# PaoPaoRobot/ygz-slam

Measured on AMD Instinct MI355X. Metric: frames/sec (extract+match+LK+local-BA), 640x480, 1000 ORB kpts; frames resident in HBM (PCIe-inclusive rate: value_with_transfers), higher is better.
Workload: dtype u8/f32/f64; 1 GPU; 2x640x480-pair pipeline: ORB extract + 256-bit Hamming BF cross-check + KLT 21x21x5 + FindDirectProjection + SparseImgAlign + local-BA 10x2000 linearise, per frame; resident_batches_per_gpu=1

## Files before the change

### ygz_slam_amd/csrc/image.hip

```cpp
#include "ygz_internal.h"
#include <limits.h>

__device__ __forceinline__ uint32_t gray1(uint32_t b, uint32_t g, uint32_t r)
{
    return (1868u * b + 9617u * g + 4899u * r + 8192u) >> 14;
}

typedef uint32_t img_u32x4 __attribute__((ext_vector_type(4)));
typedef img_u32x4 __attribute__((aligned(4))) img_u32x4u;
typedef img_u32x4 __attribute__((aligned(1))) img_u32x4b;
typedef uint32_t __attribute__((aligned(1))) img_u32b;
__global__ __launch_bounds__(256) void k_bgr2gray16(const uint8_t *__restrict__ bgr, uint8_t *__restrict__ gray,
                                                    unsigned npix, int slot_begin, uint8_t *__restrict__ pad, int width, int height)
{
    const unsigned i = blockIdx.x * 256u + threadIdx.x;
    if (i * 16u >= npix) return;
    const size_t slot = (size_t)(slot_begin + blockIdx.y);
    const uint4 *src = reinterpret_cast<const uint4 *>(bgr + slot * npix * 3u) + (size_t)i * 3u;
    const uint4 a = src[0], b = src[1], c = src[2];
    const uint32_t w[12] = { a.x, a.y, a.z, a.w, b.x, b.y, b.z, b.w, c.x, c.y, c.z, c.w };
    uint32_t out[4];
#pragma unroll
    for (int q = 0; q < 4; ++q) {
        const uint32_t w0 = w[3 * q], w1 = w[3 * q + 1], w2 = w[3 * q + 2];
        const uint32_t g0 = gray1(w0 & 255u, (w0 >> 8) & 255u, (w0 >> 16) & 255u);
        const uint32_t g1 = gray1(w0 >> 24, w1 & 255u, (w1 >> 8) & 255u);
        const uint32_t g2 = gray1((w1 >> 16) & 255u, w1 >> 24, w2 & 255u);
        const uint32_t g3 = gray1((w2 >> 8) & 255u, (w2 >> 16) & 255u, w2 >> 24);
        out[q] = g0 | (g1 << 8) | (g2 << 16) | (g3 << 24);
    }
    reinterpret_cast<uint4 *>(gray + slot * npix)[i] = make_uint4(out[0], out[1], out[2], out[3]);
    if (pad) {
        const unsigned p0 = i * 16u, y = p0 / (unsigned)width, x = p0 - y * (unsigned)width;
        const size_t pw = (size_t)KLT_PW(width), ph = (size_t)height + 2 * KLT_B;
        uint8_t *base = pad + slot * pw * ph;
        img_u32x4 v; v.x = out[0]; v.y = out[1]; v.z = out[2]; v.w = out[3];
        const uint32_t r0 = __builtin_amdgcn_perm(out[0], out[0], 0x00010203u), r1 = __builtin_amdgcn_perm(out[1], out[1], 0x00010203u),
                       r2 = __builtin_amdgcn_perm(out[2], out[2], 0x00010203u), r3 = __builtin_amdgcn_perm(out[3], out[3], 0x00010203u);
        img_u32x4 rv; rv.x = r3; rv.y = r2; rv.z = r1; rv.w = r0;
        auto store_row = [&](int r) {
            uint8_t *row = base + (size_t)r * pw;
            *reinterpret_cast<img_u32x4u *>(row + x + KLT_B) = v;
            if (x == 0u) *reinterpret_cast<img_u32x4b *>(row + KLT_B - 15) = rv;
            else if (x == 16u) {
                *reinterpret_cast<img_u32b *>(row + 5) = r0; *reinterpret_cast<img_u32b *>(row + 1) = r1; row[0] = (uint8_t)(out[2] & 255u);
            }
            if ((int)x == width - 16) *reinterpret_cast<img_u32x4b *>(row + KLT_B + width - 1) = rv;
            else if ((int)x == width - 32) {
                *reinterpret_cast<img_u32b *>(row + KLT_B + width + 15) = r3; *reinterpret_cast<img_u32b *>(row + KLT_B + width + 19) = r2;
                row[KLT_B + width + 23] = (uint8_t)(out[1] >> 24);
            }
        };
        store_row((int)y + KLT_B);
        if (y >= 1u && y <= (unsigned)KLT_B) store_row(KLT_B - (int)y);
        if ((int)y >= height - 1 - KLT_B && (int)y <= height - 2) store_row(KLT_B + 2 * (height - 1) - (int)y);
    }
}

__global__ __launch_bounds__(256) void k_bgr2gray1(const uint8_t *__restrict__ bgr, uint8_t *__restrict__ gray,
                                                   unsigned npix, int slot_begin)
{
    const unsigned i = blockIdx.x * 256u + threadIdx.x;
    if (i >= npix) return;
    const size_t slot = (size_t)(slot_begin + blockIdx.y);
    const uint8_t *s = bgr + (slot * npix + i) * 3u;
    gray[slot * npix + i] = (uint8_t)gray1(s[0], s[1], s[2]);
}

__device__ __forceinline__ int reflect101(int i, int n)
{
    if (n == 1) return 0;
    while (i < 0 || i >= n) i = (i < 0) ? -i : 2 * (n - 1) - i;
    return i;
}

#define PD_TW 64
#define PD_TH 32
#define PD_RPT (PD_TH / 4)
#define PD_SW 160
#define PD_SH (2 * PD_TH + 3)
#define PD_X0 16
__global__ __launch_bounds__(256) void k_pyr_down(const uint8_t *__restrict__ src, uint8_t *__restrict__ dst,
                                                  int sw, int sh, int dw, int dh, int slot_begin, uint8_t *__restrict__ pad, int frame_here)
{
    __shared__ __attribute__((aligned(16))) uint8_t tile[PD_SH][PD_SW];
    const size_t slot = (size_t)(slot_begin + blockIdx.z);
    const uint8_t *s = src + slot * (size_t)sw * sh;
    uint8_t *d = dst + slot * (size_t)dw * dh;
    const int dpw = KLT_PW(dw);
    uint8_t *pd = pad ? pad + slot * (size_t)dpw * (dh + 2 * KLT_B) + (size_t)KLT_B * dpw + KLT_B : nullptr;
    const int ox0 = blockIdx.x * PD_TW, oy0 = blockIdx.y * PD_TH;
    const int sx0 = 2 * ox0 - PD_X0, sy0 = 2 * oy0 - 2;
    const bool aligned = (sw & 15) == 0;
    constexpr int PD_RW = PD_SW / 16, PD_TOT = PD_SH * PD_RW, PD_N = (PD_TOT + 255) / 256;
    uint4 stage[PD_N];
#pragma unroll
    for (int k = 0; k < PD_N; ++k) {
        const int i = threadIdx.x + 256 * k;
        const int r = i / PD_RW, c16 = (i % PD_RW) * 16;
        uint4 v = make_uint4(0u, 0u, 0u, 0u);
        if (i < PD_TOT) {
            const int sy = reflect101(sy0 + r, sh), sx = sx0 + c16;
            const uint8_t *row = s + (size_t)sy * sw;
            if (aligned && sx >= 0 && sx + 15 < sw) v = *reinterpret_cast<const uint4 *>(row + sx);
            else {
                uint32_t w4[4];
#pragma unroll
                for (int q = 0; q < 4; ++q)
                    w4[q] = (uint32_t)row[reflect101(sx + 4 * q, sw)] | ((uint32_t)row[reflect101(sx + 4 * q + 1, sw)] << 8) |
                            ((uint32_t)row[reflect101(sx + 4 * q + 2, sw)] << 16) | ((uint32_t)row[reflect101(sx + 4 * q + 3, sw)] << 24);
                v = make_uint4(w4[0], w4[1], w4[2], w4[3]);
            }
        }
        stage[k] = v;
    }
#pragma unroll
    for (int k = 0; k < PD_N; ++k) {
        const int i = threadIdx.x + 256 * k;
        if (i < PD_TOT) *reinterpret_cast<uint4 *>(&tile[i / PD_RW][(i % PD_RW) * 16]) = stage[k];
    }
    __syncthreads();
    const int tx = threadIdx.x & 63, ty0 = (threadIdx.x >> 6) * PD_RPT;
    const int ox = ox0 + tx;
    int hrow[2 * PD_RPT + 3];
#pragma unroll
    for (int r = 0; r < 2 * PD_RPT + 3; ++r) {
        const uint32_t *tw = reinterpret_cast<const uint32_t *>(&tile[2 * ty0 + r][(2 * tx + PD_X0 - 2) & ~3]);
        const uint32_t d0 = tw[0], d1 = tw[1], sh = (uint32_t)((2 * tx + PD_X0 - 2) & 3);
        const uint32_t v4 = __builtin_amdgcn_alignbyte(d1, d0, sh);
        hrow[r] = (int)__builtin_amdgcn_udot4(v4, 0x04060401u, (d1 >> (8 * sh)) & 255u, false);
    }
    if (ox < dw) {
#pragma unroll
        for (int k = 0; k < PD_RPT; ++k) {
            const int oy = oy0 + ty0 + k;
            if (oy < dh) {
                const int v = hrow[2 * k] + 4 * hrow[2 * k + 1] + 6 * hrow[2 * k + 2] + 4 * hrow[2 * k + 3] + hrow[2 * k + 4];
                const uint8_t o8 = (uint8_t)((v + 128) >> 8);
                d[(size_t)oy * dw + ox] = o8;
                if (pd) {
                    pd[(size_t)oy * dpw + ox] = o8;
                    if (frame_here) {
                        const bool fl = ox >= 1 && ox <= KLT_B, fr = ox >= dw - 1 - KLT_B && ox <= dw - 2;
                        const bool ft = oy >= 1 && oy <= KLT_B, fb = oy >= dh - 1 - KLT_B && oy <= dh - 2;
                        if (fl | fr | ft | fb) {
                            const ptrdiff_t xl = -ox, xr = 2 * (dw - 1) - ox, yt = (ptrdiff_t)(-oy) * dpw, yb = (ptrdiff_t)(2 * (dh - 1) - oy) * dpw, y0 = (ptrdiff_t)oy * dpw;
                            if (fl) pd[y0 + xl] = o8;
                            if (fr) pd[y0 + xr] = o8;
                            if (ft) { pd[yt + ox] = o8; if (fl) pd[yt + xl] = o8; if (fr) pd[yt + xr] = o8; }
                            if (fb) { pd[yb + ox] = o8; if (fl) pd[yb + xl] = o8; if (fr) pd[yb + xr] = o8; }
                        }
                    }
                }
            }
        }
    }
}

struct FrameArgs {
    const uint8_t *img[YGZ_MAX_LEVELS]; uint8_t *pad[YGZ_MAX_LEVELS];
    int w[YGZ_MAX_LEVELS], h[YGZ_MAX_LEVELS];
    int first[YGZ_MAX_LEVELS], items[YGZ_MAX_LEVELS];
    int n_levels, slot_begin, full0;
};
typedef uint32_t __attribute__((aligned(1))) img_u32u;
__global__ __launch_bounds__(256) void k_klt_frame(FrameArgs A)
{
    int L = 0;
#pragma unroll
    for (int k = 1; k < YGZ_MAX_LEVELS; ++k) if (k < A.n_levels && (int)blockIdx.x >= A.first[k]) L = k;
    const int item = ((int)blockIdx.x - A.first[L]) * 256 + (int)threadIdx.x;
    if (item >= A.items[L]) return;
    const int w = A.w[L], h = A.h[L], pw = KLT_PW(w), ph = h + 2 * KLT_B, pw4 = pw >> 2;
    int y, dc;
    if (A.full0 && L == 0) { y = item / pw4; dc = item - y * pw4; }
    else {
        const int r0 = (KLT_B + w) >> 2, nr = pw4 - r0, band = KLT_B * pw4, mid = (KLT_B >> 2) + nr;
        if (item < band) { y = item / pw4; dc = item - y * pw4; }
        else if (item < 2 * band) { const int j = item - band; y = j / pw4; dc = j - y * pw4; y += KLT_B + h; }
        else {
            const int j = item - 2 * band;
            y = j / mid;
            const int c = j - y * mid;
            y += KLT_B;
            dc = c < (KLT_B >> 2) ? c : r0 + (c - (KLT_B >> 2));
        }
    }
    const size_t slot = (size_t)(A.slot_begin + (int)blockIdx.y);
    const uint8_t *row = A.img[L] + slot * (size_t)w * h + (size_t)reflect101(y - KLT_B, h) * w;
    const int x = 4 * dc - KLT_B;
    uint32_t v = 0;
    if (x >= 0 && x + 3 < w) v = *reinterpret_cast<const img_u32u *>(row + x);
    else {
#pragma unroll
        for (int k = 0; k < 4; ++k) v |= (uint32_t)row[reflect101(x + k, w)] << (8 * k);
    }
    *reinterpret_cast<uint32_t *>(A.pad[L] + slot * (size_t)pw * ph + (size_t)y * pw + 4 * dc) = v;
}

int ygz_launch_gray_pyramid(ygz_hip_ctx *ctx, int slot_begin, int n_slots, int from_bgr, int up_to_level)
{
    int rc = ygz_ensure_levels(ctx, up_to_level);
    if (rc != YGZ_OK) return rc;
    const unsigned npix = (unsigned)ctx->lw[0] * (unsigned)ctx->lh[0];
    int fuse_levels = 0;
    while (fuse_levels < up_to_level && ctx->klt_pad[fuse_levels]) ++fuse_levels;
    const bool fuse = fuse_levels > 0;
    const bool l0_framed = fuse && from_bgr && (npix & 15u) == 0 && (ctx->lw[0] & 15) == 0 && ctx->lw[0] >= 64 && ctx->lh[0] >= 2 * KLT_B + 2;
    bool framed[YGZ_MAX_LEVELS];
    for (int L = 0; L < YGZ_MAX_LEVELS; ++L) framed[L] = L == 0 ? l0_framed : (L < fuse_levels && ctx->lw[L] > KLT_B + 1 && ctx->lh[L] > KLT_B + 1);
    if (from_bgr) {
        if ((npix & 15u) == 0)
            YGZ_LAUNCH(ctx, KID_BGR2GRAY, k_bgr2gray16, dim3(ygz_div_up((int)(npix / 16), 256), n_slots), dim3(256),
                               ctx->bgr, ctx->lvl[0], npix, slot_begin, l0_framed ? ctx->klt_pad[0] : (uint8_t *)nullptr, ctx->lw[0], ctx->lh[0]);
        else
            YGZ_LAUNCH(ctx, KID_BGR2GRAY, k_bgr2gray1, dim3(ygz_div_up((int)npix, 256), n_slots), dim3(256),
                               ctx->bgr, ctx->lvl[0], npix, slot_begin);
    }
    for (int L = 1; L < up_to_level; ++L) {
        const int sw = ctx->lw[L - 1], sh = ctx->lh[L - 1], dw = ctx->lw[L], dh = ctx->lh[L];
        YGZ_LAUNCH(ctx, KID_PYR_DOWN, k_pyr_down, dim3(ygz_div_up(dw, PD_TW), ygz_div_up(dh, PD_TH), n_slots), dim3(256), ctx->lvl[L - 1], ctx->lvl[L], sw, sh, dw, dh, slot_begin,
                   L < fuse_levels ? ctx->klt_pad[L] : (uint8_t *)nullptr, framed[L] ? 1 : 0);
    }
    if (fuse) {
        FrameArgs F;
        for (int L = 0; L < YGZ_MAX_LEVELS; ++L) { F.img[L] = nullptr; F.pad[L] = nullptr; F.w[L] = F.h[L] = 0; F.first[L] = 0; F.items[L] = 0; }
        int total = 0;
        for (int L = 0; L < fuse_levels; ++L) {
            const int w = ctx->lw[L], h = ctx->lh[L], pw4 = KLT_PW(w) >> 2;
            F.img[L] = ctx->lvl[L]; F.pad[L] = ctx->klt_pad[L]; F.w[L] = w; F.h[L] = h;
            F.first[L] = total;
            F.items[L] = framed[L] ? 0 : (L == 0 ? pw4 * (h + 2 * KLT_B) : 2 * KLT_B * pw4 + h * ((KLT_B >> 2) + pw4 - ((KLT_B + w) >> 2)));
            total += ygz_div_up(F.items[L], 256);
        }
        F.n_levels = fuse_levels; F.slot_begin = slot_begin; F.full0 = 1;
        if (total > 0) YGZ_LAUNCH(ctx, KID_KLT_PAD, k_klt_frame, dim3(total, n_slots), dim3(256), F);
    }
    if ((int)ctx->pad_levels.size() >= slot_begin + n_slots)
        for (int s = slot_begin; s < slot_begin + n_slots; ++s) ctx->pad_levels[s] = (uint8_t)fuse_levels;
    YGZ_HIPCHK(ctx, hipGetLastError());
    return YGZ_OK;
}
```

### ygz_slam_amd/csrc/align.hip

```cpp
#include "ygz_internal.h"
#include <cstring>
#include <vector>
#include "../../include/ygz_exp.h"
#include "se3_dev.h"

struct Cam { float fx, fy, cx, cy; };

__device__ __forceinline__ void pixel2camera_d(const Cam &c, const double px[2], double depth, double out[3])
{
    out[0] = (px[0] - c.cx) * depth / c.fx;
    out[1] = (px[1] - c.cy) * depth / c.fy;
    out[2] = depth;
}
__device__ __forceinline__ void camera2pixel_d(const Cam &c, const double p[3], double out[2])
{
    out[0] = c.fx * p[0] / p[2] + c.cx;
    out[1] = c.fy * p[1] / p[2] + c.cy;
}

__device__ __forceinline__ float cof3(const float m[9], int i, int j)
{
    const int i1 = (i + 1) % 3, i2 = (i + 2) % 3, j1 = (j + 1) % 3, j2 = (j + 2) % 3;
    return __fsub_rn(__fmul_rn(m[3 * i1 + j1], m[3 * i2 + j2]), __fmul_rn(m[3 * i1 + j2], m[3 * i2 + j1]));
}

#define STG_ROWS 13
#define STG_DWORDS (STG_ROWS * 4)

__device__ bool align2d_core(const uint8_t *__restrict__ cur, int w, int h, const uint8_t *pwb, uint32_t *stg, int n_iter,
                             double *pu, double *pv, float *chi2_out)
{
    float H[9] = { 0, 0, 0, 0, 0, 0, 0, 0, 0 };
    for (int y = 0; y < 8; ++y)
        for (int x = 0; x < 8; ++x) {
            const int k = (y + 1) * 10 + (x + 1);
            const float jx = 0.5f * (float)((int)pwb[(k + 1) * 64] - (int)pwb[(k - 1) * 64]);
            const float jy = 0.5f * (float)((int)pwb[(k + 10) * 64] - (int)pwb[(k - 10) * 64]);
            H[0] = __fadd_rn(H[0], __fmul_rn(jx, jx)); H[1] = __fadd_rn(H[1], __fmul_rn(jx, jy)); H[2] = __fadd_rn(H[2], jx);
            H[4] = __fadd_rn(H[4], __fmul_rn(jy, jy)); H[5] = __fadd_rn(H[5], jy); H[8] = __fadd_rn(H[8], 1.0f);
        }
    H[3] = H[1]; H[6] = H[2]; H[7] = H[5];
    float Hinv[9];
    {
        const float c0 = cof3(H, 0, 0), c1 = cof3(H, 1, 0), c2 = cof3(H, 2, 0);
        const float det = __fadd_rn(__fadd_rn(__fmul_rn(c0, H[0]), __fmul_rn(c1, H[3])), __fmul_rn(c2, H[6]));
        const float invdet = __fdiv_rn(1.0f, det);
        Hinv[0] = __fmul_rn(c0, invdet); Hinv[1] = __fmul_rn(c1, invdet); Hinv[2] = __fmul_rn(c2, invdet);
        Hinv[3] = __fmul_rn(cof3(H, 0, 1), invdet); Hinv[4] = __fmul_rn(cof3(H, 1, 1), invdet); Hinv[5] = __fmul_rn(cof3(H, 2, 1), invdet);
        Hinv[6] = __fmul_rn(cof3(H, 0, 2), invdet); Hinv[7] = __fmul_rn(cof3(H, 1, 2), invdet); Hinv[8] = __fmul_rn(cof3(H, 2, 2), invdet);
    }
    float mean_diff = 0.f;
    float u = (float)*pu, v = (float)*pv;
    bool stg_ok = false;
    int sx0 = 0, sy0 = 0;
    if (stg && u == u && v == v && w >= 16 && h >= STG_ROWS) {
        const int u0 = (int)floorf(u), v0 = (int)floorf(v);
        if (!(u0 < 4 || v0 < 4 || u0 >= w - 4 || v0 >= h - 4)) {
            sx0 = min(max(u0 - 7, 0), w - 16); sy0 = min(max(v0 - 6, 0), h - STG_ROWS);
            const uint8_t *p0 = cur + (size_t)sy0 * w + sx0;
#pragma unroll
            for (int r = 0; r < STG_ROWS; ++r) {
                ygz_gptr32u q = (ygz_gptr32u)(p0 + (size_t)r * w);
#pragma unroll
                for (int d = 0; d < 4; ++d) stg[(r * 4 + d) * 64] = q[d];
            }
            stg_ok = true;
        }
    }
    const float min_update_squared = (float)(0.03 * 0.03);
    float chi2 = 0.f;
    bool converged = false;
    for (int iter = 0; iter < n_iter; ++iter) {
        chi2 = 0.f;
        if (u != u || v != v) break;
        const int u_r = (int)floorf(u), v_r = (int)floorf(v);
        if (u_r < 4 || v_r < 4 || u_r >= w - 4 || v_r >= h - 4) break;
        const float sx = __fsub_rn(u, (float)u_r), sy = __fsub_rn(v, (float)v_r);
        const float wTL = (float)((1.0 - (double)sx) * (1.0 - (double)sy));
        const float wTR = (float)((double)sx * (1.0 - (double)sy));
        const float wBL = (float)((1.0 - (double)sx) * (double)sy);
        const float wBR = __fmul_rn(sx, sy);
        float J0 = 0.f, J1 = 0.f, J2 = 0.f;
        uint32_t wl[9], wh[9], w8[9];
        const int ox = u_r - 4 - sx0, oy = v_r - 4 - sy0;
        if (stg_ok && ox >= 0 && ox <= 7 && oy >= 0 && oy <= STG_ROWS - 9) {
            const uint32_t sh = (uint32_t)(ox & 3);
            const uint32_t *sp = stg + (oy * 4 + (ox >> 2)) * 64;
#pragma unroll
            for (int r = 0; r < 9; ++r) {
                const uint32_t d0 = sp[(r * 4) * 64], d1 = sp[(r * 4 + 1) * 64], d2 = sp[(r * 4 + 2) * 64];
                wl[r] = __builtin_amdgcn_alignbyte(d1, d0, sh); wh[r] = __builtin_amdgcn_alignbyte(d2, d1, sh); w8[r] = (d2 >> (8 * sh)) & 255u;
            }
        } else {
#pragma unroll
            for (int r = 0; r < 9; ++r) {
                const uint8_t *rp = cur + (size_t)(v_r + r - 4) * w + (u_r - 4);
                ygz_load8(rp, wl[r], wh[r]); w8[r] = (uint32_t)rp[8];
            }
        }
#define WIN(r, c) ((c) < 8 ? YGZ_BYTE(wl[r], wh[r], (c) & 7) : (int)w8[r])
#pragma unroll
        for (int y = 0; y < 8; ++y) {
#pragma unroll
            for (int x = 0; x < 8; ++x) {
                const float tl = (float)WIN(y, x), tr = (float)WIN(y, x + 1), bl = (float)WIN(y + 1, x), br = (float)WIN(y + 1, x + 1);
                const float sp = __fadd_rn(__fadd_rn(__fadd_rn(__fmul_rn(wTL, tl), __fmul_rn(wTR, tr)), __fmul_rn(wBL, bl)), __fmul_rn(wBR, br));
                const int k = (y + 1) * 10 + (x + 1);
                const float refv = (float)pwb[k * 64];
                const float res = __fadd_rn(__fsub_rn(sp, refv), mean_diff);
                const float jx = 0.5f * (float)((int)pwb[(k + 1) * 64] - (int)pwb[(k - 1) * 64]);
                const float jy = 0.5f * (float)((int)pwb[(k + 10) * 64] - (int)pwb[(k - 10) * 64]);
                J0 = __fsub_rn(J0, __fmul_rn(res, jx));
                J1 = __fsub_rn(J1, __fmul_rn(res, jy));
                J2 = __fsub_rn(J2, res);
                chi2 = __fadd_rn(chi2, __fmul_rn(res, res));
            }
        }
#undef WIN
        const float up0 = __fadd_rn(__fadd_rn(__fmul_rn(Hinv[0], J0), __fmul_rn(Hinv[1], J1)), __fmul_rn(Hinv[2], J2));
        const float up1 = __fadd_rn(__fadd_rn(__fmul_rn(Hinv[3], J0), __fmul_rn(Hinv[4], J1)), __fmul_rn(Hinv[5], J2));
        const float up2 = __fadd_rn(__fadd_rn(__fmul_rn(Hinv[6], J0), __fmul_rn(Hinv[7], J1)), __fmul_rn(Hinv[8], J2));
        u = __fadd_rn(u, up0); v = __fadd_rn(v, up1); mean_diff = __fadd_rn(mean_diff, up2);
        if (__fadd_rn(__fmul_rn(up0, up0), __fmul_rn(up1, up1)) < min_update_squared) { converged = true; break; }
    }
    *pu = (double)u; *pv = (double)v;
    if (chi2_out) *chi2_out = chi2;
    return converged && chi2 < 20000.f;
}

static __device__ __forceinline__ void warp_affine_lds(const double Am[4], const uint8_t *img, int rw, int rh, const double px_ref[2], int Lr, int sl,
                                                       uint8_t *pwb)
{
    const double det = Am[0] * Am[3] - Am[2] * Am[1];
    const double invdet = 1.0 / det;
    const double R0 = Am[3] * invdet, R1 = -Am[1] * invdet, R2 = -Am[2] * invdet, R3 = Am[0] * invdet;
    const double rx = px_ref[0] / (double)(1 << Lr), ry = px_ref[1] / (double)(1 << Lr);
    const double sc = (double)(1 << sl);
    for (int y = 0; y < 10; ++y) {
        double xx[10], yy[10];
        uint32_t top[10], bot[10];
        bool inb[10];
#pragma unroll
        for (int x = 0; x < 10; ++x) {
            double ppx = (double)(x - 5), ppy = (double)(y - 5);
            ppx *= sc; ppy *= sc;
            const double qx = (R0 * ppx + R1 * ppy) + rx, qy = (R2 * ppx + R3 * ppy) + ry;
            inb[x] = !(qx < 0 || qy < 0 || qx >= rw - 1 || qy >= rh - 1);
            xx[x] = qx - floor(qx); yy[x] = qy - floor(qy);
            const uint8_t *d = inb[x] ? img + (size_t)((int)qy) * rw + (int)qx : img;
            top[x] = *reinterpret_cast<const ygz_u16u *>(d); bot[x] = *reinterpret_cast<const ygz_u16u *>(d + rw);
        }
#pragma unroll
        for (int x = 0; x < 10; ++x) {
            const int d00 = (int)(top[x] & 255u), d01 = (int)(top[x] >> 8), d10 = (int)(bot[x] & 255u), d11 = (int)(bot[x] >> 8);
            const uint8_t val = (uint8_t)((1 - xx[x]) * (1 - yy[x]) * d00 + xx[x] * (1 - yy[x]) * d01 + (1 - xx[x]) * yy[x] * d10 + xx[x] * yy[x] * d11);
            pwb[(y * 10 + x) * 64] = inb[x] ? val : (uint8_t)0;
        }
    }
}

struct FdpArgs {
    const uint8_t *lvl[YGZ_MAX_LEVELS];
    size_t sstride[YGZ_MAX_LEVELS];
    int w[YGZ_MAX_LEVELS], h[YGZ_MAX_LEVELS];
    int n_levels, cells, n_pairs;
    Cam cam;
    const int32_t *pair_q, *pair_t, *trk_n;
    const double *pair_T;
    const double *trk_px, *trk_depth; const int32_t *trk_level;
    double *px_cur; int32_t *search_level; uint8_t *ok;
    const uint8_t *cand;
    int prio;
};

static __device__ __forceinline__ bool fdp_core(const FdpArgs &A, int ref_slot, int cur_slot, const double *Tr7, const double *Tc7,
                                                const double px_ref[2], double depth, int Lr, uint8_t *pwb, uint32_t *stg, double px_cur[2],
                                                int *sl_out)
{
    double pt_ref[3];
    pixel2camera_d(A.cam, px_ref, depth, pt_ref);
    Se3 T_ref, T_cur, Tri, TCR;
    for (int k = 0; k < 4; ++k) { T_ref.q[k] = Tr7[k]; T_cur.q[k] = Tc7[k]; }
    for (int k = 0; k < 3; ++k) { T_ref.t[k] = Tr7[4 + k]; T_cur.t[k] = Tc7[4 + k]; }
    se3_inv_d(&T_ref, &Tri);
    se3_mul_d(&T_cur, &Tri, &TCR);
    double Am[4];
    {
        double pw[3], pdu[3], pdv[3], q[3], pc[2], pu[2], pv[2];
        se3_act_d(&Tri, pt_ref, pw);
        const double s = (double)(1 << Lr);
        const double pxu[2] = { px_ref[0] + 4.0 * s, px_ref[1] + 0.0 * s };
        const double pxv[2] = { px_ref[0] + 0.0 * s, px_ref[1] + 4.0 * s };
        pixel2camera_d(A.cam, pxu, pt_ref[2], pdu);
        pixel2camera_d(A.cam, pxv, pt_ref[2], pdv);
        se3_act_d(&TCR, pw, q);  camera2pixel_d(A.cam, q, pc);
        se3_act_d(&TCR, pdu, q); camera2pixel_d(A.cam, q, pu);
        se3_act_d(&TCR, pdv, q); camera2pixel_d(A.cam, q, pv);
        Am[0] = (pu[0] - pc[0]) / 4; Am[2] = (pu[1] - pc[1]) / 4;
        Am[1] = (pv[0] - pc[0]) / 4; Am[3] = (pv[1] - pc[1]) / 4;
    }
    int sl = 0;
    {
        double D = Am[0] * Am[3] - Am[2] * Am[1];
        while (D > 3.0 && sl < A.n_levels - 1) { sl += 1; D *= 0.25; }
    }
    warp_affine_lds(Am, A.lvl[Lr] + (size_t)ref_slot * A.sstride[Lr], A.w[Lr], A.h[Lr], px_ref, Lr, sl, pwb);
    const int cw = A.w[sl], ch = A.h[sl];
    const uint8_t *cur = A.lvl[sl] + (size_t)cur_slot * A.sstride[sl];
    double u = px_cur[0] / (double)(1 << sl), v = px_cur[1] / (double)(1 << sl);
    const bool good = align2d_core(cur, cw, ch, pwb, stg, 10, &u, &v, nullptr);
    const double ox = u * (double)(1 << sl), oy = v * (double)(1 << sl);
    px_cur[0] = ox; px_cur[1] = oy;
    *sl_out = sl;
    const bool inframe = ox >= 10 && ox < A.w[0] - 10 && oy >= 10 && oy < A.h[0] - 10;
    return inframe && good;
}

__global__ __launch_bounds__(64) void k_find_direct_projection(FdpArgs A)
{
    __shared__ uint8_t pwb_all[100 * 64];
    __shared__ uint32_t stg_all[STG_DWORDS * 64];
    int bx, pair;
    ygz_raise_prio(A.prio);
    if (!ygz_xcd_remap(A.n_pairs, bx, pair)) return;
    const int ii = bx * 64 + threadIdx.x;
    if (ii >= A.trk_n[pair]) return;
    const size_t i = (size_t)pair * A.cells + ii;
    const double depth = A.trk_depth[i];
    if (depth < 0 || (A.cand && !A.cand[i])) { A.ok[i] = 0; A.search_level[i] = 0; return; }
    const double px_ref[2] = { A.trk_px[2 * i], A.trk_px[2 * i + 1] };
    double px_cur[2] = { A.px_cur[2 * i], A.px_cur[2 * i + 1] };
    int sl;
    const bool ok = fdp_core(A, A.pair_t[pair], A.pair_q[pair], A.pair_T + 14 * (size_t)pair, A.pair_T + 14 * (size_t)pair + 7,
                             px_ref, depth, A.trk_level[i], pwb_all + threadIdx.x, stg_all + threadIdx.x, px_cur, &sl);
    A.px_cur[2 * i] = px_cur[0]; A.px_cur[2 * i + 1] = px_cur[1];
    A.search_level[i] = sl;
    A.ok[i] = (uint8_t)ok;
}

struct LmapArgs {
    FdpArgs F;
    int cur_slot, P, C, K;
    const double *T_cur;
    const double *pos_world; const uint8_t *point_bad;
    const int32_t *kf_slot; const double *kf_T;
    const int32_t *cand_point, *cand_kf, *cand_level; const double *cand_px_ref;
    uint8_t *in_view; double *px_proj; int32_t *match_cand; double *px_match; int32_t *match_level;
    double *cand_px; int32_t *cand_sl; uint8_t *cand_ok;
    int given_px;
};

__global__ __launch_bounds__(256) void k_lmap_project(LmapArgs A)
{
    const int p = blockIdx.x * 256 + threadIdx.x;
    if (p >= A.P) return;
    A.match_cand[p] = 0x7fffffff; A.match_level[p] = 0;
    A.px_match[2 * p] = 0.0; A.px_match[2 * p + 1] = 0.0;
    if (A.given_px) { A.in_view[p] = 1; return; }
    double px[2] = { 0.0, 0.0 };
    bool vis = false;
    if (!(A.point_bad && A.point_bad[p])) {
        Se3 T;
        for (int k = 0; k < 4; ++k) T.q[k] = A.T_cur[k];
        for (int k = 0; k < 3; ++k) T.t[k] = A.T_cur[4 + k];
        const double pw[3] = { A.pos_world[3 * (size_t)p], A.pos_world[3 * (size_t)p + 1], A.pos_world[3 * (size_t)p + 2] };
        double pc[3];
        se3_act_d(&T, pw, pc);
        camera2pixel_d(A.F.cam, pc, px);
        vis = !(pc[2] < 0) && px[0] >= 20 && px[0] < A.F.w[0] - 20 && px[1] >= 20 && px[1] < A.F.h[0] - 20;
    }
// ... 854 lines not shown
```

Baseline: 106,000 frames/s.

## Fuse BGR-to-gray conversion with first pyramid level downsample into one kernel

Adds k_gray_level1, which converts BGR (or reads gray) for a 128x64 tile plus halo, writes level 0 and its framed KLT pad, and computes level 1 from shared memory in the same kernel. This removes one launch and the global re-read of level 0 when the grid fits within n_cu*8 groups. The level-0 tile is loaded and converted redundantly in the halo regions. Pad address math also switches from size_t to 32-bit offsets to trim integer work.

```diff
diff --git a/ygz_slam_amd/csrc/image.hip b/ygz_slam_amd/csrc/image.hip
--- a/ygz_slam_amd/csrc/image.hip
+++ b/ygz_slam_amd/csrc/image.hip
@@ -4,12 +4,53 @@
 __device__ __forceinline__ uint32_t gray1(uint32_t b, uint32_t g, uint32_t r)
 {
     return (1868u * b + 9617u * g + 4899u * r + 8192u) >> 14;
+}
+
+__device__ __forceinline__ uint32_t gray4(uint32_t w0, uint32_t w1, uint32_t w2)
+{
+    const uint32_t g0 = gray1(w0 & 255u, (w0 >> 8) & 255u, (w0 >> 16) & 255u);
+    const uint32_t g1 = gray1(w0 >> 24, w1 & 255u, (w1 >> 8) & 255u);
+    const uint32_t g2 = gray1((w1 >> 16) & 255u, w1 >> 24, w2 & 255u);
+    const uint32_t g3 = gray1((w2 >> 8) & 255u, (w2 >> 16) & 255u, w2 >> 24);
+    return g0 | (g1 << 8) | (g2 << 16) | (g3 << 24);
 }
 
 typedef uint32_t img_u32x4 __attribute__((ext_vector_type(4)));
 typedef img_u32x4 __attribute__((aligned(4))) img_u32x4u;
 typedef img_u32x4 __attribute__((aligned(1))) img_u32x4b;
 typedef uint32_t __attribute__((aligned(1))) img_u32b;
+__device__ __forceinline__ void store_framed16(uint8_t *base, size_t pw, unsigned x, unsigned y, int width, int height, const uint32_t out[4])
+{
+    img_u32x4 v; v.x = out[0]; v.y = out[1]; v.z = out[2]; v.w = out[3];
+    const uint32_t r0 = __builtin_amdgcn_perm(out[0], out[0], 0x00010203u), r1 = __builtin_amdgcn_perm(out[1], out[1], 0x00010203u),
+                   r2 = __builtin_amdgcn_perm(out[2], out[2], 0x00010203u), r3 = __builtin_amdgcn_perm(out[3], out[3], 0x00010203u);
+    img_u32x4 rv; rv.x = r3; rv.y = r2; rv.z = r1; rv.w = r0;
+    const uint32_t pw32 = (uint32_t)pw, wd = (uint32_t)width;
+    auto store_row = [&](int r) {
+        const uint32_t o = (uint32_t)r * pw32;
+        *reinterpret_cast<img_u32x4u *>(base + (o + x + KLT_B)) = v;
+        if (x == 0u) *reinterpret_cast<img_u32x4b *>(base + (o + (KLT_B - 15))) = rv;
+        else if (x == 16u) {
+            *reinterpret_cast<img_u32b *>(base + (o + 5)) = r0; *reinterpret_cast<img_u32b *>(base + (o + 1)) = r1; base[o] = (uint8_t)(out[2] & 255u);
+        }
+        if (x == wd - 16u) *reinterpret_cast<img_u32x4b *>(base + (o + KLT_B + wd - 1)) = rv;
+        else if (x == wd - 32u) {
+            *reinterpret_cast<img_u32b *>(base + (o + KLT_B + wd + 15)) = r3; *reinterpret_cast<img_u32b *>(base + (o + KLT_B + wd + 19)) = r2;
+            base[o + KLT_B + wd + 23] = (uint8_t)(out[1] >> 24);
+        }
+    };
+    store_row((int)y + KLT_B);
+    if (y >= 1u && y <= (unsigned)KLT_B) store_row(KLT_B - (int)y);
+    if ((int)y >= height - 1 - KLT_B && (int)y <= height - 2) store_row(KLT_B + 2 * (height - 1) - (int)y);
+}
+
+__device__ __forceinline__ void gray16(const uint4 a, const uint4 b, const uint4 c, uint32_t out[4])
+{
+    const uint32_t w[12] = { a.x, a.y, a.z, a.w, b.x, b.y, b.z, b.w, c.x, c.y, c.z, c.w };
+#pragma unroll
+    for (int q = 0; q < 4; ++q) out[q] = gray4(w[3 * q], w[3 * q + 1], w[3 * q + 2]);
+}
+
 __global__ __launch_bounds__(256) void k_bgr2gray16(const uint8_t *__restrict__ bgr, uint8_t *__restrict__ gray,
                                                     unsigned npix, int slot_begin, uint8_t *__restrict__ pad, int width, int height)
 {
@@ -18,42 +59,13 @@
     const size_t slot = (size_t)(slot_begin + blockIdx.y);
     const uint4 *src = reinterpret_cast<const uint4 *>(bgr + slot * npix * 3u) + (size_t)i * 3u;
     const uint4 a = src[0], b = src[1], c = src[2];
-    const uint32_t w[12] = { a.x, a.y, a.z, a.w, b.x, b.y, b.z, b.w, c.x, c.y, c.z, c.w };
     uint32_t out[4];
-#pragma unroll
-    for (int q = 0; q < 4; ++q) {
-        const uint32_t w0 = w[3 * q], w1 = w[3 * q + 1], w2 = w[3 * q + 2];
-        const uint32_t g0 = gray1(w0 & 255u, (w0 >> 8) & 255u, (w0 >> 16) & 255u);
-        const uint32_t g1 = gray1(w0 >> 24, w1 & 255u, (w1 >> 8) & 255u);
-        const uint32_t g2 = gray1((w1 >> 16) & 255u, w1 >> 24, w2 & 255u);
-        const uint32_t g3 = gray1((w2 >> 8) & 255u, (w2 >> 16) & 255u, w2 >> 24);
-        out[q] = g0 | (g1 << 8) | (g2 << 16) | (g3 << 24);
-    }
+    gray16(a, b, c, out);
     reinterpret_cast<uint4 *>(gray + slot * npix)[i] = make_uint4(out[0], out[1], out[2], out[3]);
     if (pad) {
         const unsigned p0 = i * 16u, y = p0 / (unsigned)width, x = p0 - y * (unsigned)width;
         const size_t pw = (size_t)KLT_PW(width), ph = (size_t)height + 2 * KLT_B;
-        uint8_t *base = pad + slot * pw * ph;
-        img_u32x4 v; v.x = out[0]; v.y = out[1]; v.z = out[2]; v.w = out[3];
-        const uint32_t r0 = __builtin_amdgcn_perm(out[0], out[0], 0x00010203u), r1 = __builtin_amdgcn_perm(out[1], out[1], 0x00010203u),
-                       r2 = __builtin_amdgcn_perm(out[2], out[2], 0x00010203u), r3 = __builtin_amdgcn_perm(out[3], out[3], 0x00010203u);
-        img_u32x4 rv; rv.x = r3; rv.y = r2; rv.z = r1; rv.w = r0;
-        auto store_row = [&](int r) {
-            uint8_t *row = base + (size_t)r * pw;
-            *reinterpret_cast<img_u32x4u *>(row + x + KLT_B) = v;
-            if (x == 0u) *reinterpret_cast<img_u32x4b *>(row + KLT_B - 15) = rv;
-            else if (x == 16u) {
-                *reinterpret_cast<img_u32b *>(row + 5) = r0; *reinterpret_cast<img_u32b *>(row + 1) = r1; row[0] = (uint8_t)(out[2] & 255u);
-            }
-            if ((int)x == width - 16) *reinterpret_cast<img_u32x4b *>(row + KLT_B + width - 1) = rv;
-            else if ((int)x == width - 32) {
-                *reinterpret_cast<img_u32b *>(row + KLT_B + width + 15) = r3; *reinterpret_cast<img_u32b *>(row + KLT_B + width + 19) = r2;
-                row[KLT_B + width + 23] = (uint8_t)(out[1] >> 24);
-            }
-        };
-        store_row((int)y + KLT_B);
-        if (y >= 1u && y <= (unsigned)KLT_B) store_row(KLT_B - (int)y);
-        if ((int)y >= height - 1 - KLT_B && (int)y <= height - 2) store_row(KLT_B + 2 * (height - 1) - (int)y);
+        store_framed16(pad + slot * pw * ph, pw, x, y, width, height, out);
     }
 }
 
@@ -80,6 +92,53 @@
 #define PD_SW 160
 #define PD_SH (2 * PD_TH + 3)
 #define PD_X0 16
+__device__ __forceinline__ void store_level_px(uint8_t *__restrict__ d, uint8_t *__restrict__ pb, int dpw, int dw, int dh, int ox, int oy, uint8_t o8, int frame_here)
+{
+    d[(uint32_t)(oy * dw + ox)] = o8;
+    if (!pb) return;
+    const uint32_t px = (uint32_t)(ox + KLT_B), py = (uint32_t)((oy + KLT_B) * dpw);
+    pb[py + px] = o8;
+    if (!frame_here) return;
+    const bool fl = ox >= 1 && ox <= KLT_B, fr = ox >= dw - 1 - KLT_B && ox <= dw - 2;
+    const bool ft = oy >= 1 && oy <= KLT_B, fb = oy >= dh - 1 - KLT_B && oy <= dh - 2;
+    if (fl | fr | ft | fb) {
+        const uint32_t xl = (uint32_t)(KLT_B - ox), xr = (uint32_t)(KLT_B + 2 * (dw - 1) - ox);
+        const uint32_t yt = (uint32_t)((KLT_B - oy) * dpw), yb = (uint32_t)((KLT_B + 2 * (dh - 1) - oy) * dpw);
+        if (fl) pb[py + xl] = o8;
+        if (fr) pb[py + xr] = o8;
+        if (ft) { pb[yt + px] = o8; if (fl) pb[yt + xl] = o8; if (fr) pb[yt + xr] = o8; }
+        if (fb) { pb[yb + px] = o8; if (fl) pb[yb + xl] = o8; if (fr) pb[yb + xr] = o8; }
+    }
+}
+
+__device__ __forceinline__ int hsum5(const uint8_t *img, int a)
+{
+    const uint32_t *tw = reinterpret_cast<const uint32_t *>(img + (a & ~3));
+    const uint32_t d0 = tw[0], d1 = tw[1], sh = (uint32_t)(a & 3);
+    const uint32_t v4 = __builtin_amdgcn_alignbyte(d1, d0, sh);
+    return (int)__builtin_amdgcn_udot4(v4, 0x04060401u, (d1 >> (8 * sh)) & 255u, false);
+}
+
+__device__ __forceinline__ void pyr_down_tile(const uint8_t (*tile)[PD_SW], int ox0, int oy0, int dw, int dh,
+                                              uint8_t *__restrict__ d, uint8_t *__restrict__ pb, int dpw, int frame_here)
+{
+    const int tx = threadIdx.x & 63, ty0 = (threadIdx.x >> 6) * PD_RPT;
+    const int ox = ox0 + tx;
+    int hrow[2 * PD_RPT + 3];
+#pragma unroll
+    for (int r = 0; r < 2 * PD_RPT + 3; ++r) hrow[r] = hsum5(&tile[2 * ty0 + r][0], 2 * tx + PD_X0 - 2);
+    if (ox < dw) {
+#pragma unroll
+        for (int k = 0; k < PD_RPT; ++k) {
+            const int oy = oy0 + ty0 + k;
+            if (oy < dh) {
+                const int v = hrow[2 * k] + 4 * hrow[2 * k + 1] + 6 * hrow[2 * k + 2] + 4 * hrow[2 * k + 3] + hrow[2 * k + 4];
+                store_level_px(d, pb, dpw, dw, dh, ox, oy, (uint8_t)((v + 128) >> 8), frame_here);
+            }
+        }
+    }
+}
+
 __global__ __launch_bounds__(256) void k_pyr_down(const uint8_t *__restrict__ src, uint8_t *__restrict__ dst,
                                                   int sw, int sh, int dw, int dh, int slot_begin, uint8_t *__restrict__ pad, int frame_here)
 {
@@ -88,7 +147,7 @@
     const uint8_t *s = src + slot * (size_t)sw * sh;
     uint8_t *d = dst + slot * (size_t)dw * dh;
     const int dpw = KLT_PW(dw);
-    uint8_t *pd = pad ? pad + slot * (size_t)dpw * (dh + 2 * KLT_B) + (size_t)KLT_B * dpw + KLT_B : nullptr;
+    uint8_t *pd = pad ? pad + slot * (size_t)dpw * (dh + 2 * KLT_B) : nullptr;
     const int ox0 = blockIdx.x * PD_TW, oy0 = blockIdx.y * PD_TH;
     const int sx0 = 2 * ox0 - PD_X0, sy0 = 2 * oy0 - 2;
     const bool aligned = (sw & 15) == 0;
@@ -120,41 +179,105 @@
         if (i < PD_TOT) *reinterpret_cast<uint4 *>(&tile[i / PD_RW][(i % PD_RW) * 16]) = stage[k];
     }
     __syncthreads();
-    const int tx = threadIdx.x & 63, ty0 = (threadIdx.x >> 6) * PD_RPT;
-    const int ox = ox0 + tx;
-    int hrow[2 * PD_RPT + 3];
-#pragma unroll
-    for (int r = 0; r < 2 * PD_RPT + 3; ++r) {
-        const uint32_t *tw = reinterpret_cast<const uint32_t *>(&tile[2 * ty0 + r][(2 * tx + PD_X0 - 2) & ~3]);
-        const uint32_t d0 = tw[0], d1 = tw[1], sh = (uint32_t)((2 * tx + PD_X0 - 2) & 3);
-        const uint32_t v4 = __builtin_amdgcn_alignbyte(d1, d0, sh);
-        hrow[r] = (int)__builtin_amdgcn_udot4(v4, 0x04060401u, (d1 >> (8 * sh)) & 255u, false);
-    }
-    if (ox < dw) {
-#pragma unroll
-        for (int k = 0; k < PD_RPT; ++k) {
-            const int oy = oy0 + ty0 + k;
-            if (oy < dh) {
-                const int v = hrow[2 * k] + 4 * hrow[2 * k + 1] + 6 * hrow[2 * k + 2] + 4 * hrow[2 * k + 3] + hrow[2 * k + 4];
-                const uint8_t o8 = (uint8_t)((v + 128) >> 8);
-                d[(size_t)oy * dw + ox] = o8;
-                if (pd) {
-                    pd[(size_t)oy * dpw + ox] = o8;
-                    if (frame_here) {
-                        const bool fl = ox >= 1 && ox <= KLT_B, fr = ox >= dw - 1 - KLT_B && ox <= dw - 2;
-                        const bool ft = oy >= 1 && oy <= KLT_B, fb = oy >= dh - 1 - KLT_B && oy <= dh - 2;
-                        if (fl | fr | ft | fb) {
-                            const ptrdiff_t xl = -ox, xr = 2 * (dw - 1) - ox, yt = (ptrdiff_t)(-oy) * dpw, yb = (ptrdiff_t)(2 * (dh - 1) - oy) * dpw, y0 = (ptrdiff_t)oy * dpw;
-                            if (fl) pd[y0 + xl] = o8;
-                            if (fr) pd[y0 + xr] = o8;
-                            if (ft) { pd[yt + ox] = o8; if (fl) pd[yt + xl] = o8; if (fr) pd[yt + xr] = o8; }
-                            if (fb) { pd[yb + ox] = o8; if (fl) pd[yb + xl] = o8; if (fr) pd[yb + xr] = o8; }
-                        }
-                    }
+    pyr_down_tile(tile, ox0, oy0, dw, dh, d, pd, dpw, frame_here);
+}
+
+#define GL_HALO_ROWS 3
+#define GL_ROW_ITEMS (GL_HALO_ROWS * (2 * PD_TW / 16))
+#define GL_HALO_ITEMS (GL_ROW_ITEMS + 2 * PD_SH)
+#define GL_GROUPS_PER_CU 8
+template <bool BGR>
+__global__ __launch_bounds__(256) void k_gray_level1(const uint8_t *__restrict__ src, uint8_t *__restrict__ gray, uint8_t *__restrict__ lvl1,
+                                                     int w, int h, int dw, int dh, int slot_begin,
+                                                     uint8_t *__restrict__ pad0, uint8_t *__restrict__ pad1, int frame1)
+{
+    static_assert(2 * PD_TW == 128 && 2 * PD_TH == 64 && PD_X0 == 16 && PD_SW >= 2 * PD_TW + PD_X0 + 4 && GL_HALO_ITEMS <= 256, "tile geometry");
+    __shared__ __attribute__((aligned(16))) uint8_t tile[PD_SH][PD_SW];
+    constexpr int BPP = BGR ? 3 : 1, NV = BGR ? 3 : 1;
+    const size_t slot = (size_t)(slot_begin + blockIdx.z), npix = (size_t)w * h;
+    const uint8_t *s = src + slot * npix * BPP;
+    uint8_t *g0 = BGR ? gray + slot * npix : nullptr;
+    const int ox0 = blockIdx.x * PD_TW, oy0 = blockIdx.y * PD_TH, x0 = 2 * ox0, y0 = 2 * oy0;
+    const size_t pw0 = (size_t)KLT_PW(w);
+    uint8_t *p0 = pad0 ? pad0 + slot * pw0 * ((size_t)h + 2 * KLT_B) : nullptr;
+    auto load16 = [&](int ry, int x, uint4 (&v)[NV]) {
+        const uint4 *q = reinterpret_cast<const uint4 *>(s + (uint32_t)((ry * w + x) * BPP));
+#pragma unroll
+        for (int k = 0; k < NV; ++k) v[k] = q[k];
+    };
+    auto conv16 = [&](const uint4 (&v)[NV], uint32_t out[4]) {
+        if constexpr (BGR) gray16(v[0], v[1], v[2], out);
+        else { out[0] = v[0].x; out[1] = v[0].y; out[2] = v[0].z; out[3] = v[0].w; }
+    };
+    const int cx = x0 + 16 * (threadIdx.x & 7), cr = threadIdx.x >> 3;
+    uint4 cv[2][NV];
+    bool cok[2];
+#pragma unroll
+    for (int k = 0; k < 2; ++k) {
+        const int y = y0 + cr + 32 * k;
+        cok[k] = cx < w && y <= h + 1;
+        if (cok[k]) load16(y < h ? y : 2 * (h - 1) - y, cx, cv[k]);
+    }
+    const int t = threadIdx.x;
+    const bool row_item = t < GL_ROW_ITEMS, col_item = !row_item && t < GL_HALO_ITEMS;
+    int hr = 0, hx = 0;
+    bool hok = false, hfast = false;
+    uint4 hv[NV];
+    uint32_t hw4[NV] = {};
+    if (row_item) {
+        hr = (t >> 3) < 2 ? (t >> 3) : PD_SH - 1;
+        hx = x0 + 16 * (t & 7);
+        const int y = y0 - 2 + hr;
+        hok = hx < w && y <= h + 1;
+        if (hok) load16(reflect101(y, h), hx, hv);
+    } else if (col_item) {
+        const int j = t - GL_ROW_ITEMS;
+        hr = j >> 1;
+        hx = (j & 1) ? min(x0 + 2 * PD_TW, w) : x0 - 4;
+        const int y = y0 - 2 + hr;
+        hok = y <= h + 1;
+        hfast = hx >= 0 && hx + 3 < w;
+        if (hok) {
+            const uint8_t *row = s + (uint32_t)(reflect101(y, h) * w * BPP);
+            if (hfast) {
+#pragma unroll
+                for (int k = 0; k < NV; ++k) hw4[k] = reinterpret_cast<const uint32_t *>(row + (size_t)hx * BPP)[k];
+            } else {
+                uint32_t g = 0;
+#pragma unroll
+                for (int q = 0; q < 4; ++q) {
+                    const uint8_t *px = row + (size_t)reflect101(hx + q, w) * BPP;
+                    g |= (BGR ? gray1(px[0], px[BPP > 1 ? 1 : 0], px[BPP > 1 ? 2 : 0]) : (uint32_t)px[0]) << (8 * q);
                 }
+                hw4[0] = g;
             }
         }
     }
+#pragma unroll
+    for (int k = 0; k < 2; ++k) {
+        if (!cok[k]) continue;
+        const int y = y0 + cr + 32 * k;
+        uint32_t out[4];
+        conv16(cv[k], out);
+        *reinterpret_cast<uint4 *>(&tile[cr + 32 * k + 2][cx - x0 + PD_X0]) = make_uint4(out[0], out[1], out[2], out[3]);
+        if (y < h) {
+            if constexpr (BGR) *reinterpret_cast<uint4 *>(g0 + (uint32_t)(y * w + cx)) = make_uint4(out[0], out[1], out[2], out[3]);
+            if (p0) store_framed16(p0, pw0, (unsigned)cx, (unsigned)y, w, h, out);
+        }
+    }
+    if (row_item && hok) {
+        uint32_t out[4];
+        conv16(hv, out);
+        *reinterpret_cast<uint4 *>(&tile[hr][hx - x0 + PD_X0]) = make_uint4(out[0], out[1], out[2], out[3]);
+    } else if (col_item && hok) {
+        uint32_t g = hw4[0];
+        if constexpr (BGR) { if (hfast) g = gray4(hw4[0], hw4[1], hw4[2]); }
+        *reinterpret_cast<uint32_t *>(&tile[hr][hx - x0 + PD_X0]) = g;
+    }
+    __syncthreads();
+    const int dpw = KLT_PW(dw);
+    uint8_t *pd = pad1 ? pad1 + slot * (size_t)dpw * (dh + 2 * KLT_B) : nullptr;
+    pyr_down_tile(tile, ox0, oy0, dw, dh, lvl1 + slot * (size_t)dw * dh, pd, dpw, frame1);
 }
 
 struct FrameArgs {
@@ -206,10 +329,22 @@
     int fuse_levels = 0;
     while (fuse_levels < up_to_level && ctx->klt_pad[fuse_levels]) ++fuse_levels;
     const bool fuse = fuse_levels > 0;
-    const bool l0_framed = fuse && from_bgr && (npix & 15u) == 0 && (ctx->lw[0] & 15) == 0 && ctx->lw[0] >= 64 && ctx->lh[0] >= 2 * KLT_B + 2;
+    const bool l0_geom = (ctx->lw[0] & 15) == 0 && ctx->lw[0] >= 64 && ctx->lh[0] >= 2 * KLT_B + 2;
+    const bool fused01 = l0_geom && up_to_level >= 2 &&
+                         (long)ygz_div_up(ctx->lw[1], PD_TW) * ygz_div_up(ctx->lh[1], PD_TH) * n_slots <= (long)ctx->n_cu * GL_GROUPS_PER_CU;
+    const bool l0_framed = fuse && l0_geom && (from_bgr || fused01);
     bool framed[YGZ_MAX_LEVELS];
     for (int L = 0; L < YGZ_MAX_LEVELS; ++L) framed[L] = L == 0 ? l0_framed : (L < fuse_levels && ctx->lw[L] > KLT_B + 1 && ctx->lh[L] > KLT_B + 1);
-    if (from_bgr) {
+    auto pad_of = [&](int L) { return L < fuse_levels ? ctx->klt_pad[L] : (uint8_t *)nullptr; };
+    if (fused01) {
+        const dim3 grid(ygz_div_up(ctx->lw[1], PD_TW), ygz_div_up(ctx->lh[1], PD_TH), n_slots);
+        if (from_bgr)
+            YGZ_LAUNCH(ctx, KID_BGR2GRAY, k_gray_level1<true>, grid, dim3(256), ctx->bgr, ctx->lvl[0], ctx->lvl[1], ctx->lw[0], ctx->lh[0], ctx->lw[1], ctx->lh[1],
+                       slot_begin, pad_of(0), pad_of(1), framed[1] ? 1 : 0);
+        else
+            YGZ_LAUNCH(ctx, KID_BGR2GRAY, k_gray_level1<false>, grid, dim3(256), ctx->lvl[0], (uint8_t *)nullptr, ctx->lvl[1], ctx->lw[0], ctx->lh[0], ctx->lw[1], ctx->lh[1],
+                       slot_begin, pad_of(0), pad_of(1), framed[1] ? 1 : 0);
+    } else if (from_bgr) {
         if ((npix & 15u) == 0)
             YGZ_LAUNCH(ctx, KID_BGR2GRAY, k_bgr2gray16, dim3(ygz_div_up((int)(npix / 16), 256), n_slots), dim3(256),
                                ctx->bgr, ctx->lvl[0], npix, slot_begin, l0_framed ? ctx->klt_pad[0] : (uint8_t *)nullptr, ctx->lw[0], ctx->lh[0]);
@@ -217,10 +352,10 @@
             YGZ_LAUNCH(ctx, KID_BGR2GRAY, k_bgr2gray1, dim3(ygz_div_up((int)npix, 256), n_slots), dim3(256),
                                ctx->bgr, ctx->lvl[0], npix, slot_begin);
     }
-    for (int L = 1; L < up_to_level; ++L) {
+    for (int L = fused01 ? 2 : 1; L < up_to_level; ++L) {
         const int sw = ctx->lw[L - 1], sh = ctx->lh[L - 1], dw = ctx->lw[L], dh = ctx->lh[L];
         YGZ_LAUNCH(ctx, KID_PYR_DOWN, k_pyr_down, dim3(ygz_div_up(dw, PD_TW), ygz_div_up(dh, PD_TH), n_slots), dim3(256), ctx->lvl[L - 1], ctx->lvl[L], sw, sh, dw, dh, slot_begin,
-                   L < fuse_levels ? ctx->klt_pad[L] : (uint8_t *)nullptr, framed[L] ? 1 : 0);
+                   pad_of(L), framed[L] ? 1 : 0);
     }
     if (fuse) {
         FrameArgs F;
```

Measured after the change: 106,000 frames/s. About the same (-0.0%).

## Vectorize align2d inner loop with packed f32/f16 math and precomputed gradients

Applied to the files above, without the earlier changes.

Precomputes the reference-patch gradients once, outside the iteration loop, as packed fp16 pairs. The Hessian is built with integer sdot2 accumulations, and the reference pixels are kept packed in registers. The per-iteration residual and Jacobian loop now uses packed float2 arithmetic and v_fma_mix instructions, which mix f16 gradients with f32 residuals. This removes repeated LDS byte loads and scalar FLOPs per iteration, at the cost of more register pressure and possible rounding-order differences in the accumulations.

```diff
diff --git a/ygz_slam_amd/csrc/align.hip b/ygz_slam_amd/csrc/align.hip
--- a/ygz_slam_amd/csrc/align.hip
+++ b/ygz_slam_amd/csrc/align.hip
@@ -26,19 +26,56 @@
 
 #define STG_ROWS 13
 #define STG_DWORDS (STG_ROWS * 4)
+typedef _Float16 a2d_h2 __attribute__((ext_vector_type(2)));
+typedef float a2d_f2 __attribute__((ext_vector_type(2)));
+typedef short a2d_s2 __attribute__((ext_vector_type(2)));
+template <int HI> __device__ __forceinline__ float a2d_mul_mix(float a, a2d_h2 g)
+{
+    float r;
+    if (HI) asm("v_fma_mix_f32 %0, %1, %2, %3 op_sel:[0,1,0] op_sel_hi:[0,1,0]" : "=v"(r) : "v"(a), "v"(g), "s"(-0.0f));
+    else    asm("v_fma_mix_f32 %0, %1, %2, %3 op_sel:[0,0,0] op_sel_hi:[0,1,0]" : "=v"(r) : "v"(a), "v"(g), "s"(-0.0f));
+    return r;
+}
 
 __device__ bool align2d_core(const uint8_t *__restrict__ cur, int w, int h, const uint8_t *pwb, uint32_t *stg, int n_iter,
                              double *pu, double *pv, float *chi2_out)
 {
-    float H[9] = { 0, 0, 0, 0, 0, 0, 0, 0, 0 };
-    for (int y = 0; y < 8; ++y)
-        for (int x = 0; x < 8; ++x) {
-            const int k = (y + 1) * 10 + (x + 1);
-            const float jx = 0.5f * (float)((int)pwb[(k + 1) * 64] - (int)pwb[(k - 1) * 64]);
-            const float jy = 0.5f * (float)((int)pwb[(k + 10) * 64] - (int)pwb[(k - 10) * 64]);
-            H[0] = __fadd_rn(H[0], __fmul_rn(jx, jx)); H[1] = __fadd_rn(H[1], __fmul_rn(jx, jy)); H[2] = __fadd_rn(H[2], jx);
-            H[4] = __fadd_rn(H[4], __fmul_rn(jy, jy)); H[5] = __fadd_rn(H[5], jy); H[8] = __fadd_rn(H[8], 1.0f);
-        }
+    a2d_h2 gdx[32], gdy[32];
+    uint32_t rf[16];
+    int sxx = 0, sxy = 0, syy = 0;
+    a2d_s2 sx2 = { 0, 0 }, sy2 = { 0, 0 };
+    {
+#define PK2(k0) ((uint32_t)pwb[(k0) * 64] | ((uint32_t)pwb[((k0) + 1) * 64] << 16) | 0x66006600u)
+        uint32_t hx[8][5], hy[10][4];
+#pragma unroll
+        for (int y = 0; y < 8; ++y)
+#pragma unroll
+            for (int c = 0; c < 5; ++c) hx[y][c] = PK2((y + 1) * 10 + 2 * c);
+#pragma unroll
+        for (int r = 0; r < 10; ++r)
+#pragma unroll
+            for (int j = 0; j < 4; ++j) hy[r][j] = PK2(r * 10 + 2 * j + 1);
+#undef PK2
+#pragma unroll
+        for (int y = 0; y < 8; ++y) {
+#pragma unroll
+            for (int j = 0; j < 4; ++j) {
+                const a2d_s2 dx = __builtin_bit_cast(a2d_s2, hx[y][j + 1]) - __builtin_bit_cast(a2d_s2, hx[y][j]);
+                const a2d_s2 dy = __builtin_bit_cast(a2d_s2, hy[y + 2][j]) - __builtin_bit_cast(a2d_s2, hy[y][j]);
+                gdx[y * 4 + j] = __builtin_bit_cast(a2d_h2, hx[y][j + 1]) - __builtin_bit_cast(a2d_h2, hx[y][j]);
+                gdy[y * 4 + j] = __builtin_bit_cast(a2d_h2, hy[y + 2][j]) - __builtin_bit_cast(a2d_h2, hy[y][j]);
+                sxx = __builtin_amdgcn_sdot2(dx, dx, sxx, false); sxy = __builtin_amdgcn_sdot2(dx, dy, sxy, false);
+                syy = __builtin_amdgcn_sdot2(dy, dy, syy, false);
+                sx2 += dx; sy2 += dy;
+            }
+            rf[y * 2] = __builtin_amdgcn_perm(hy[y + 1][1], hy[y + 1][0], 0x06040200u);
+            rf[y * 2 + 1] = __builtin_amdgcn_perm(hy[y + 1][3], hy[y + 1][2], 0x06040200u);
+        }
+    }
+    const int sx1 = (int)sx2.x + (int)sx2.y, sy1 = (int)sy2.x + (int)sy2.y;
+    float H[9];
+    H[0] = 0.25f * (float)sxx; H[1] = 0.25f * (float)sxy; H[2] = 0.5f * (float)sx1;
+    H[4] = 0.25f * (float)syy; H[5] = 0.5f * (float)sy1; H[8] = 64.0f;
     H[3] = H[1]; H[6] = H[2]; H[7] = H[5];
     float Hinv[9];
     {
@@ -80,7 +117,8 @@
         const float wTR = (float)((double)sx * (1.0 - (double)sy));
         const float wBL = (float)((1.0 - (double)sx) * (double)sy);
         const float wBR = __fmul_rn(sx, sy);
-        float J0 = 0.f, J1 = 0.f, J2 = 0.f;
+        a2d_f2 J01 = { 0.f, 0.f };
+        float J2 = 0.f;
         uint32_t wl[9], wh[9], w8[9];
         const int ox = u_r - 4 - sx0, oy = v_r - 4 - sy0;
         if (stg_ok && ox >= 0 && ox <= 7 && oy >= 0 && oy <= STG_ROWS - 9) {
@@ -100,22 +138,39 @@
         }
 #define WIN(r, c) ((c) < 8 ? YGZ_BYTE(wl[r], wh[r], (c) & 7) : (int)w8[r])
 #pragma unroll
-        for (int y = 0; y < 8; ++y) {
-#pragma unroll
-            for (int x = 0; x < 8; ++x) {
-                const float tl = (float)WIN(y, x), tr = (float)WIN(y, x + 1), bl = (float)WIN(y + 1, x), br = (float)WIN(y + 1, x + 1);
-                const float sp = __fadd_rn(__fadd_rn(__fadd_rn(__fmul_rn(wTL, tl), __fmul_rn(wTR, tr)), __fmul_rn(wBL, bl)), __fmul_rn(wBR, br));
-                const int k = (y + 1) * 10 + (x + 1);
-                const float refv = (float)pwb[k * 64];
-                const float res = __fadd_rn(__fsub_rn(sp, refv), mean_diff);
-                const float jx = 0.5f * (float)((int)pwb[(k + 1) * 64] - (int)pwb[(k - 1) * 64]);
-                const float jy = 0.5f * (float)((int)pwb[(k + 10) * 64] - (int)pwb[(k - 10) * 64]);
-                J0 = __fsub_rn(J0, __fmul_rn(res, jx));
-                J1 = __fsub_rn(J1, __fmul_rn(res, jy));
-                J2 = __fsub_rn(J2, res);
-                chi2 = __fadd_rn(chi2, __fmul_rn(res, res));
+        for (int p = 0; p < 32; ++p) { asm volatile("" : "+v"(gdx[p])); asm volatile("" : "+v"(gdy[p])); }
+#pragma unroll
+        for (int p = 0; p < 16; ++p) asm volatile("" : "+v"(rf[p]));
+        a2d_f2 fe[2][4], fo[2][4];
+#pragma unroll
+        for (int r = 0; r < 9; ++r) {
+            float f[9];
+#pragma unroll
+            for (int c = 0; c < 9; ++c) f[c] = (float)WIN(r, c);
+#pragma unroll
+            for (int j = 0; j < 4; ++j) {
+                fe[r & 1][j] = a2d_f2{ f[2 * j], f[2 * j + 1] }; fo[r & 1][j] = a2d_f2{ f[2 * j + 1], f[2 * j + 2] };
+                asm("" : "+v"(fe[r & 1][j])); asm("" : "+v"(fo[r & 1][j]));
             }
-        }
+            if (r == 0) continue;
+            const int y = r - 1;
+#pragma unroll
+            for (int j = 0; j < 4; ++j) {
+                const a2d_f2 sp = (((wTL * fe[y & 1][j]) + (wTR * fo[y & 1][j])) + (wBL * fe[r & 1][j])) + (wBR * fo[r & 1][j]);
+                const uint32_t rw = rf[y * 2 + (j >> 1)] >> (16 * (j & 1));
+                const a2d_f2 refv = { (float)(rw & 255u), (float)((rw >> 8) & 255u) };
+                a2d_f2 nres = (refv - sp) - mean_diff;
+                asm("" : "+v"(nres));
+                a2d_f2 sq = nres * nres;
+                asm("" : "+v"(sq));
+                const int p = y * 4 + j;
+                J01 = J01 + a2d_f2{ a2d_mul_mix<0>(nres.x, gdx[p]), a2d_mul_mix<0>(nres.x, gdy[p]) };
+                J2 = __fadd_rn(J2, nres.x); chi2 = __fadd_rn(chi2, sq.x);
+                J01 = J01 + a2d_f2{ a2d_mul_mix<1>(nres.y, gdx[p]), a2d_mul_mix<1>(nres.y, gdy[p]) };
+                J2 = __fadd_rn(J2, nres.y); chi2 = __fadd_rn(chi2, sq.y);
+            }
+        }
+        const float J0 = __fmul_rn(0.5f, J01.x), J1 = __fmul_rn(0.5f, J01.y);
 #undef WIN
         const float up0 = __fadd_rn(__fadd_rn(__fmul_rn(Hinv[0], J0), __fmul_rn(Hinv[1], J1)), __fmul_rn(Hinv[2], J2));
         const float up1 = __fadd_rn(__fadd_rn(__fmul_rn(Hinv[3], J0), __fmul_rn(Hinv[4], J1)), __fmul_rn(Hinv[5], J2));
```

After: 104,000 frames/s before, 104,200 frames/s after, median of 6. About the same (+0.2%).
